# gmlwns2000/sea-attention

Measured on AMD Instinct MI355X. Metric: tokens/sec + achieved HBM GB/s, OPT-1.3B SEA T=4096 k=64, 1/2/4/8 MI355X, higher is better.
Workload: dtype bf16

## Files before the change

include/sea_hip.h:

```cpp
#ifndef SEA_HIP_H
#define SEA_HIP_H

#include <stdint.h>

#ifdef __cplusplus
extern "C" {
#endif

#define SEA_ABI_VERSION 6

enum sea_dtype { SEA_F32 = 0, SEA_F16 = 1, SEA_BF16 = 2 };

enum sea_error {
  SEA_OK = 0,
  SEA_EINVAL = -1,
  SEA_EUNSUPPORTED = -2,
  SEA_ELAUNCH = -3
};

typedef void* sea_stream_t;

int sea_version(void);
const char* sea_last_error(void);

// ... 42 lines not shown

int sea_csr_elmul(const float* in_values, float* out_values,
                  const void* other, int dtype, const int64_t* other_strides ,
                  int64_t N, int64_t H, int64_t T_dst, int64_t T_src,
                  const void* crow, const void* col, int idx_bytes, int64_t col_stride_n,
                  sea_stream_t stream);

int sea_csr_spmm(const float* values, const void* v, int dtype,
                 int64_t N, int64_t H, int64_t T_dst, int64_t T_src, int64_t D,
                 const int64_t* v_strides ,
                 const void* crow, const void* col, int idx_bytes, int64_t col_stride_n,
                 const int32_t* head_off,
                 float* out, sea_stream_t stream);

enum sea_attn_path { SEA_ATTN_AUTO = 0, SEA_ATTN_GATHER = 1, SEA_ATTN_TILE = 2, SEA_ATTN_KEYRANGE = 3 };
int sea_sparse_attention(const void* q, const void* k, const void* v, int dtype,
                         int64_t N, int64_t H, int64_t T_dst, int64_t T_src, int64_t D,
                         const int64_t* q_strides, const int64_t* k_strides, const int64_t* v_strides,
                         const int32_t* crow, const int32_t* col, int64_t col_stride_n,
                         const int32_t* head_off,
                         const float* row_scale,
                         const void* avg, const int64_t* avg_strides,
                         const float* mix,
                         void* out, int out_dtype, const int64_t* out_strides,
                         float* probs_out, int64_t probs_stride_n,
                         const uint8_t* block_path,
                         int flags,
                         const uint32_t* bits, int64_t T_m, int is_causal, int max_k, int write_cols,
                         const int32_t* t_src_dev,
                         int64_t t_src_stride,
// ... 120 lines not shown
```

sea-attention_amd/_lib.py:

```python
import ctypes
import os
from ctypes import c_int, c_int32, c_int64, c_void_p, c_char_p, POINTER

import torch

from . import _build

SEA_F32, SEA_F16, SEA_BF16 = 0, 1, 2
ABI_VERSION = 6
_DTYPES = {torch.float32: SEA_F32, torch.float16: SEA_F16, torch.bfloat16: SEA_BF16}

_lib = None

i64 = c_int64
ptr = c_void_p
_i64p = POINTER(c_int64)

_SIGNATURES = {
    "sea_version": ([], c_int),
    "sea_last_error": ([], c_char_p),
    "sea_topk_select": ([ptr, c_int, i64, i64, i64, i64, i64, i64, i64, ptr, i64, i64, c_int, c_int,
                         ptr, ptr, ptr, ptr, ptr], c_int),
    "sea_mask_to_bits": ([ptr, c_int, i64, i64, i64, i64, i64, i64, i64, i64, c_int, c_int,
                          ptr, ptr, ptr, ptr], c_int),
# ... 46 lines not shown
    "sea_decode_append_rows": ([c_int, i64, i64, i64, i64, i64, i64, i64, i64, ptr, ptr, _i64p, _i64p, ptr, ptr, i64, i64, i64,
                                ptr, i64, ptr, i64, i64, ptr, i64, ptr, i64, ptr, ptr, ptr, i64, c_int32, c_int32, c_int32, ptr],
                               c_int),
    "sea_performer_avg_supported": ([i64, i64, c_int], c_int),
    "sea_performer_plan": ([i64, i64, i64, i64, i64, c_int, _i64p, _i64p], c_int),
}

EXPORTED_SYMBOLS = tuple(_SIGNATURES)


def library_path():
    return _build.LIB_PATH


SEA_ATTN_AUTO, SEA_ATTN_GATHER, SEA_ATTN_TILE, SEA_ATTN_KEYRANGE = 0, 1, 2, 3
SEA_OK, SEA_EINVAL, SEA_EUNSUPPORTED = 0, -1, -2


def load(build_if_missing=True):
    global _lib
    if _lib is not None:
        return _lib
    override = os.environ.get("SEA_HIP_LIB")
    if override:
        if not os.path.exists(override):
            raise RuntimeError(f"SEA_HIP_LIB={override} does not exist")
        path = override
    else:
        path = _build.LIB_PATH
        if _build.is_stale():
# ... 92 lines not shown
```

sea-attention_amd/csrc/sea_attn.hip:

```cpp
#include "sea_attn.hpp"

namespace sea {

template <typename T, typename TO, int LPR, int U, bool WP>
__global__ __launch_bounds__(256) void sparse_attn_kernel(AttnParams p) {
  constexpr int VEC = Elem<T>::VEC;
  constexpr int KPI = 64 / LPR;
  int pair, tb;
  if (!map_block(p.N * p.H, p.TB, &pair, &tb)) return;
  const int n = pair / p.H, h = pair - n * p.H;
  const int t = tb * 4 + (threadIdx.x >> 6);
  if (t >= p.T_dst) return;
  if (kernel_is_idle(p)) return;
  const int lane = threadIdx.x & 63;
  const int grp = lane / LPR, sub = lane - grp * LPR;
  const bool dact = sub * VEC < p.D;

  const T* qp = reinterpret_cast<const T*>(p.q) + n * p.qs[0] + h * p.qs[1] + t * p.qs[2] + sub * VEC;
  const T* kb = reinterpret_cast<const T*>(p.k) + n * p.ks[0] + h * p.ks[1] + sub * VEC;
  const T* vb = reinterpret_cast<const T*>(p.v) + n * p.vs[0] + h * p.vs[1] + sub * VEC;

  uint4 qraw = make_uint4(0, 0, 0, 0);
  if (dact) qraw = *reinterpret_cast<const uint4*>(qp);
  const int row_beg = p.crow[(int64_t)n * (p.T_dst + 1) + t];
// ... 84 lines not shown
      const T* ap = reinterpret_cast<const T*>(p.avg) + n * p.as[0] + h * p.as[1] + t * p.as[2] + sub * VEC;
      float af[VEC];
      unpack16<T>(*reinterpret_cast<const uint4*>(ap), af);
#pragma unroll
      for (int j = 0; j < VEC; ++j) o[j] = o[j] * a + (1.0f - a) * af[j];
    }
    TO* op = reinterpret_cast<TO*>(p.out) + n * p.os[0] + h * p.os[1] + t * p.os[2] + sub * VEC;
    store_frag<TO, VEC>(op, o);
  }
}

__device__ inline int slot_length(const AttnParams& p, int n, int h, int tn) {
  if (tn >= p.T_dst) return -1;
  const int32_t* hon = p.head_off + ((int64_t)n * p.T_dst + tn) * (p.H + 1);
  return hon[h + 1] - hon[h];
}

template <int LPR, int RPB, bool DEC = false>
__device__ inline void fused_expand(const AttnParams& p, int n, int h, int tt, bool rowok, int gi, int sub, int beg, int end,
                                    int hcol, int t_src, int* s_keys, int* lbase_out, bool* fits_out, int* total_out) {
  __shared__ int s_glen[RPB];
  const int mylen = end - beg;
  if (sub == 0) s_glen[gi] = mylen;
  __syncthreads();
  int bef = 0, tot = 0;
#pragma unroll
  for (int r = sub; r < RPB; r += LPR) {
    const int v_ = s_glen[r];
    tot += v_;
    bef += r < gi ? v_ : 0;
// ... 76 lines not shown
    }
    asm volatile("" ::"v"(sink));
  }
  __syncthreads();
}

template <bool FUSE>
__device__ inline int entry_column(const AttnParams& p, const int32_t* col, int n, int ec, int beg, const int* s_keys, int lbase, bool fits) {
  if (FUSE && fits) return s_keys[lbase + ec - beg];
  if (FUSE) return __hip_atomic_load(p.col_w + n * p.col_stride_n + ec, __ATOMIC_RELAXED, __HIP_MEMORY_SCOPE_AGENT);
  return col[ec];
}

constexpr int SEA_ATTN_WARM_ROWS = 8;

template <typename T, typename TO, int LPR, int U, bool WP, int NWB = 4, bool FUSE = false, bool DEC = false>
__global__ __launch_bounds__(NWB * 64, (FUSE && !DEC && sizeof(T) == 2 && !WP) ? 8 : 1) void sparse_attn_rows_kernel(AttnParams p) {
  static_assert(!DEC || FUSE, "the decode form is a fused form");
  constexpr int VEC = Elem<T>::VEC;
  constexpr int RPW = 64 / LPR;
  constexpr int RPB = NWB * RPW;
  int pair, tb;
  if (kernel_is_idle(p) || !map_block(p.N * p.H, p.TB, &pair, &tb)) return;
  const int n = pair / p.H;
  const int h = (pair - n * p.H + n) % p.H;
  const int lane = threadIdx.x & 63;
  const int grp = lane / LPR, sub = lane - grp * LPR;
  const int gi = (int)(threadIdx.x >> 6) * RPW + grp;
  bool rowok;
  const int t = tb * RPB + rows_by_length<LPR, RPB>(slot_length(p, n, h, tb * RPB + gi), gi, sub, &rowok);
  const bool dact = sub * VEC < p.D;
  const int tt = t < p.T_dst ? t : p.T_dst - 1;
  const int sube = dact ? sub : 0;

  const char* kbase = reinterpret_cast<const char*>(reinterpret_cast<const T*>(p.k) + n * p.ks[0] + h * p.ks[1]);
  const char* vbase = reinterpret_cast<const char*>(reinterpret_cast<const T*>(p.v) + n * p.vs[0] + h * p.vs[1]);
  const uint32_t kst = (uint32_t)p.ks[2] * (uint32_t)sizeof(T), vst = (uint32_t)p.vs[2] * (uint32_t)sizeof(T);
  const uint32_t lane_off = (uint32_t)(sube * VEC) * (uint32_t)sizeof(T);

  uint4 qraw = make_uint4(0, 0, 0, 0);
  if (dact) qraw = *reinterpret_cast<const uint4*>(reinterpret_cast<const T*>(p.q) + n * p.qs[0] + h * p.qs[1] +
                                                  (int64_t)tt * p.qs[2] + sub * VEC);
  const int row_beg = p.crow[(int64_t)n * (p.T_dst + 1) + tt];
  const int32_t* ho = p.head_off + ((int64_t)n * p.T_dst + tt) * (p.H + 1);
  const int beg = row_beg + ho[h];
// ... 135 lines not shown
}
template <> __device__ inline float tail_dot<__half>(uint32_t q, uint32_t k, float d) {
  return __builtin_amdgcn_fdot2(__builtin_bit_cast(sea_h2, q), __builtin_bit_cast(sea_h2, k), d, false);
}
template <typename T> __device__ inline void unpack2(uint32_t r, float* f);
template <> __device__ inline void unpack2<__hip_bfloat16>(uint32_t r, float* f) {
  f[0] = __uint_as_float(r << 16); f[1] = __uint_as_float(r & 0xffff0000u);
}
template <> __device__ inline void unpack2<__half>(uint32_t r, float* f) {
  const float2 t = __half22float2(__builtin_bit_cast(__half2, r));
  f[0] = t.x; f[1] = t.y;
}
template <typename TO> __device__ inline void store2(TO* dst, float a, float b) { *reinterpret_cast<uint32_t*>(dst) = pack2<TO>(a, b); }
template <> __device__ inline void store2<float>(float* dst, float a, float b) { *reinterpret_cast<float2*>(dst) = make_float2(a, b); }

template <typename T, typename TO, int U, bool WP, int NWB = 4, bool FUSE = false, bool DEC = false>
__global__ __launch_bounds__(NWB * 64) void sparse_attn_rows80_kernel(AttnParams p) {
  static_assert(!DEC || FUSE, "the decode form is a fused form");
  constexpr int LPR = 8, VEC = 8, XT = 2, DM = LPR * VEC;
  constexpr int RPW = 64 / LPR, RPB = NWB * RPW;
  int pair, tb;
  if (kernel_is_idle(p) || !map_block(p.N * p.H, p.TB, &pair, &tb)) return;
  const int n = pair / p.H;
  const int h = (pair - n * p.H + n) % p.H;
  const int lane = threadIdx.x & 63;
  const int grp = lane / LPR, sub = lane - grp * LPR;
  const int gi = (int)(threadIdx.x >> 6) * RPW + grp;
  bool rowok;
  const int t = tb * RPB + rows_by_length<LPR, RPB>(slot_length(p, n, h, tb * RPB + gi), gi, sub, &rowok);
  const int tt = t < p.T_dst ? t : p.T_dst - 1;

  const char* kbase = reinterpret_cast<const char*>(reinterpret_cast<const T*>(p.k) + n * p.ks[0] + h * p.ks[1]);
  const char* vbase = reinterpret_cast<const char*>(reinterpret_cast<const T*>(p.v) + n * p.vs[0] + h * p.vs[1]);
  const uint32_t kst = (uint32_t)p.ks[2] * (uint32_t)sizeof(T), vst = (uint32_t)p.vs[2] * (uint32_t)sizeof(T);
  const uint32_t off_m = (uint32_t)(sub * VEC) * (uint32_t)sizeof(T);
  const uint32_t off_x = (uint32_t)(DM + sub * XT) * (uint32_t)sizeof(T);

  const T* qrow = reinterpret_cast<const T*>(p.q) + n * p.qs[0] + h * p.qs[1] + (int64_t)tt * p.qs[2];
  const uint4 qraw = *reinterpret_cast<const uint4*>(qrow + sub * VEC);
  const uint32_t qx = *reinterpret_cast<const uint32_t*>(qrow + DM + sub * XT);
  const int row_beg = p.crow[(int64_t)n * (p.T_dst + 1) + tt];
  const int32_t* ho = p.head_off + ((int64_t)n * p.T_dst + tt) * (p.H + 1);
  const int beg = row_beg + ho[h];
  const int end = rowok ? row_beg + ho[h + 1] : beg;
// ... 499 lines not shown
      } else if (lpr == 8) {
        constexpr int CH = 256, DL = 64;
        hipLaunchKernelGGL((sparse_attn_decode1_kernel<T, TO, 8, false, false, WP>), dim3((unsigned)NH), dim3(256), CH * 8 + CH + CH * DL * 2, s, p);
      } else {
        constexpr int CH = 128, DL = 128;
        hipLaunchKernelGGL((sparse_attn_decode1_kernel<T, TO, 16, false, false, WP>), dim3((unsigned)NH), dim3(256), CH * 8 + CH + CH * DL * 2, s, p);
      }
      return SEA_OK;
    }
  }
  if (p.table) return SEA_EUNSUPPORTED;
  if constexpr (sizeof(T) == 2) {
    if (p.D == 80 && small) {
      const int rpb = 8 * 8;
      p.TB = (p.T_dst + rpb - 1) / rpb;
      const int64_t blocks = (int64_t)8 * ((NH + 7) / 8) * p.TB;
      if (p.bits && p.t_src_dev) {
        hipLaunchKernelGGL((sparse_attn_rows80_kernel<T, TO, 4, WP, 8, true, true>), dim3((unsigned)blocks), dim3(512), p.fuse_cap * (int)sizeof(int), s, p);
      } else if (p.bits) hipLaunchKernelGGL((sparse_attn_rows80_kernel<T, TO, 4, WP, 8, true>), dim3((unsigned)blocks), dim3(512), p.fuse_cap * (int)sizeof(int), s, p);
      else hipLaunchKernelGGL((sparse_attn_rows80_kernel<T, TO, 4, WP, 8>), dim3((unsigned)blocks), dim3(512), 0, s, p);
      return SEA_OK;
    }
  }
  if (lpr <= 16 && small) {
    const int nwb = lpr == 4 ? 4 : 8;
    const int rpb = nwb * (64 / lpr);
    p.TB = (p.T_dst + rpb - 1) / rpb;
    const int64_t blocks = (int64_t)8 * ((NH + 7) / 8) * p.TB;
    dim3 grid((unsigned)blocks), block(nwb * 64);
    if (p.bits) {
      if (lpr == 4) return SEA_EUNSUPPORTED;
      const int lds = p.fuse_cap * (int)sizeof(int);
      if (p.t_src_dev) {
        if (lpr == 8) hipLaunchKernelGGL((sparse_attn_rows_kernel<T, TO, 8, 4, WP, 8, true, true>), grid, block, lds, s, p);
        else hipLaunchKernelGGL((sparse_attn_rows_kernel<T, TO, 16, 4, WP, 8, true, true>), grid, block, lds, s, p);
        return SEA_OK;
      }
      if (lpr == 8) hipLaunchKernelGGL((sparse_attn_rows_kernel<T, TO, 8, 4, WP, 8, true>), grid, block, lds, s, p);
      else hipLaunchKernelGGL((sparse_attn_rows_kernel<T, TO, 16, 4, WP, 8, true>), grid, block, lds, s, p);
      return SEA_OK;
    }
    switch (lpr) {
      case 4: hipLaunchKernelGGL((sparse_attn_rows_kernel<T, TO, 4, 4, WP, 4>), grid, block, 0, s, p); break;
      case 8: hipLaunchKernelGGL((sparse_attn_rows_kernel<T, TO, 8, 4, WP, 8>), grid, block, 0, s, p); break;
      default: hipLaunchKernelGGL((sparse_attn_rows_kernel<T, TO, 16, 4, WP, 8>), grid, block, 0, s, p); break;
    }
    return SEA_OK;
  }
  if (p.bits) return SEA_EUNSUPPORTED;
  const int64_t blocks = (int64_t)8 * ((NH + 7) / 8) * p.TB;
  dim3 grid((unsigned)blocks), block(256);
  switch (lpr) {
// ... 53 lines not shown
  SEA_REQUIRE(dtype == SEA_F32 || dtype == SEA_F16 || dtype == SEA_BF16, SEA_EINVAL, "%s: bad dtype %d", name, dtype);
  return SEA_OK;
}

extern "C" int sea_sparse_attention(const void* q, const void* k, const void* v, int dtype, int64_t N, int64_t H,
                                    int64_t T_dst, int64_t T_src, int64_t D, const int64_t* q_strides,
                                    const int64_t* k_strides, const int64_t* v_strides, const int32_t* crow,
                                    const int32_t* col, int64_t col_stride_n, const int32_t* head_off,
                                    const float* row_scale, const void* avg, const int64_t* avg_strides,
                                    const float* mix, void* out, int out_dtype, const int64_t* out_strides,
                                    float* probs_out, int64_t probs_stride_n, const uint8_t* block_path, int flags,
                                    const uint32_t* bits, int64_t T_m, int is_causal, int max_k, int write_cols,
                                    const int32_t* t_src_dev, int64_t t_src_stride, const int32_t* block_table,
                                    int64_t table_stride, int64_t page_rows, sea_stream_t stream) {
  const char* nm = "sea_sparse_attention";
  const bool keyrange = (flags & 0xff) == SEA_ATTN_KEYRANGE;
  KeyRangeParams kr = {nullptr, 0, 0, 0};
  if (keyrange) {
    SEA_REQUIRE(bits != nullptr, SEA_EUNSUPPORTED, "%s: the key-range form is a fused form (bits is NULL)", nm);
    SEA_REQUIRE(t_src_dev == nullptr && block_table == nullptr && t_src_stride == 0, SEA_EUNSUPPORTED,
                "%s: the key-range form has no decode or paged form (t_src_dev / block_table)", nm);
    SEA_REQUIRE(write_cols == 0, SEA_EUNSUPPORTED, "%s: the key-range form writes no columns (write_cols must be 0)", nm);
    SEA_REQUIRE(N > 0 && H > 0 && T_dst > 0 && T_src > 0 && D > 0, SEA_EINVAL, "%s: bad shape", nm);
    SEA_REQUIRE(dtype == SEA_F32 ? (D == 32 || D == 64) : (D == 64 || D == 128), SEA_EUNSUPPORTED,
                "%s: the key-range form takes 16-bit D in {64, 128} or fp32 D in {32, 64} (dtype %d, D=%lld)", nm, dtype, (long long)D);
    const int64_t rk = (flags >> 16) & 0x7fff;
    SEA_REQUIRE(rk > 0, SEA_EINVAL, "%s: the key-range form needs range_keys (1 .. 32767) in bits 16..30 of flags", nm);
    const int64_t nr = (T_src + rk - 1) / rk;
    SEA_REQUIRE(nr <= 64, SEA_EUNSUPPORTED, "%s: the key-range form takes at most 64 ranges (%lld keys in ranges of %lld: %lld)", nm,
                (long long)T_src, (long long)rk, (long long)nr);
// ... 58 lines not shown
  p.crow = crow; p.col = col; p.col_stride_n = col_stride_n; p.head_off = head_off;
  p.row_scale = row_scale; p.avg = avg; p.mix = mix; p.out = out;
  p.probs = probs_out; p.probs_stride_n = probs_stride_n;
  p.sel = nullptr; p.sel_want = 0; p.TB16 = (int)((T_dst + 15) / 16);
  p.sel_count = nullptr; p.sel_total = (int)(N * H * p.TB16);
  p.sel_num = D >= 128 ? 13 : 1; p.sel_den = D >= 128 ? 20 : 2;
  p.bits = bits; p.col_w = const_cast<int32_t*>(col); p.T_m = (int)T_m; p.W = (int)((H * T_m + 31) / 32);
  p.max_k = max_k; p.is_causal = is_causal;
  p.fuse_cap = 8192;
  p.write_cols = write_cols != 0;
  p.t_src_dev = t_src_dev;
  SEA_REQUIRE(t_src_stride >= 0 && t_src_stride * N < (1ll << 31), SEA_EINVAL, "%s: bad T_src stride %lld", nm,
              (long long)t_src_stride);
  p.t_src_stride = (int)t_src_stride;
  p.table = block_table; p.table_stride = (int)table_stride; p.page_shift = block_table ? __builtin_ctzll(page_rows) : 0;
  if (t_src_dev) {
    SEA_REQUIRE(bits != nullptr && T_dst <= SEA_ATTN_WARM_ROWS, SEA_EUNSUPPORTED,
                "%s: the decode form takes T_dst <= %d rows per sequence", nm, SEA_ATTN_WARM_ROWS);
    SEA_REQUIRE(probs_out == nullptr || probs_stride_n >= col_stride_n, SEA_EINVAL,
                "%s: the decode form's probs_out needs probs_stride_n >= col_stride_n (%lld < %lld)", nm,
                (long long)probs_stride_n, (long long)col_stride_n);
  }
  if (bits) {
    SEA_REQUIRE(path != SEA_ATTN_TILE && block_path == nullptr, SEA_EUNSUPPORTED, "%s: the fused interpolation runs on the gather kernels", nm);
    SEA_REQUIRE(T_m > 0 && T_m % 32 == 0 && max_k > 0, SEA_EUNSUPPORTED, "%s: fused interpolation needs T_m %% 32 == 0", nm);
    if (t_src_dev) SEA_REQUIRE(H * T_src < (1ll << 31), SEA_EUNSUPPORTED, "%s: the decode form needs int32 ids (H*T_cap < 2^31)", nm);
    else SEA_REQUIRE(H * T_src < (1ll << 24), SEA_EUNSUPPORTED, "%s: H*T_src must stay below 2^24 (fp32-exact ids)", nm);
  }
  p.TB = (int)((T_dst + 3) / 4);
  hipStream_t s = (hipStream_t)stream;
// ... 120 lines not shown
```

sea-attention_amd/csrc/sea_attn.hpp:

```cpp
#pragma once
#include "sea_common.hpp"

namespace sea {

struct AttnParams {
  const void *q, *k, *v;
  int64_t qs[3], ks[3], vs[3];
  int N, H, T_dst, T_src, D;
  const int32_t* crow;
  const int32_t* col;
  int64_t col_stride_n;
  const int32_t* head_off;
  const float* row_scale;
  const void* avg;
  int64_t as[3];
  const float* mix;
  void* out;
  int64_t os[3];
  float* probs;
  int64_t probs_stride_n;
  const uint8_t* sel;
  int sel_want, TB16;
  const int32_t* sel_count;
  int sel_total, sel_num, sel_den;
  int TB;
  const uint32_t* bits;
  int32_t* col_w;
  int T_m, W, max_k, is_causal, fuse_cap;
  int write_cols;
  const int32_t* t_src_dev;
  int t_src_stride;
  const int32_t* table;
  int table_stride, page_shift;
};

template <typename TO, int VEC> __device__ inline void store_frag(TO* dst, const float* f);
template <> __device__ inline void store_frag<float, 4>(float* dst, const float* f) {
  *reinterpret_cast<float4*>(dst) = make_float4(f[0], f[1], f[2], f[3]);
}
template <> __device__ inline void store_frag<float, 8>(float* dst, const float* f) {
  *reinterpret_cast<float4*>(dst) = make_float4(f[0], f[1], f[2], f[3]);
  *reinterpret_cast<float4*>(dst + 4) = make_float4(f[4], f[5], f[6], f[7]);
}
template <> __device__ inline void store_frag<__hip_bfloat16, 8>(__hip_bfloat16* dst, const float* f) {
  union { uint4 u; __hip_bfloat16 h[8]; } r;
#pragma unroll
  for (int i = 0; i < 8; ++i) r.h[i] = __float2bfloat16(f[i]);
  *reinterpret_cast<uint4*>(dst) = r.u;
// ... 130 lines not shown
```

sea-attention_amd/perlin_attention/attention.py:

```python
import math
import os
import warnings
from typing import NamedTuple, Optional

import torch
import torch.nn.functional as F
from torch import nn

from ..utils import get_bench
from .config import PerlinAttentionConfig, get_default_config
from .modules import CausalConv2d, KeepRes, UpsampleFP32
from .performer import FastAttention, ProjectionUpdater
from . import ops

timer = lambda name: get_bench().region(name)
mem = lambda name: get_bench().mem_region(name)
_C8_DECLINED = set()


def _safe_to(t, d):
    return t.to(d) if isinstance(t, torch.Tensor) else t


class PerlinAttentionOutput(NamedTuple):
    loss: torch.Tensor
    context_layer: torch.Tensor
    partial_attention_probs: torch.Tensor
    partial_attention_mask: torch.Tensor
    estimated_attention_probs_m: torch.Tensor
    estimated_attention_probs: torch.Tensor
    dense_attention_probs: torch.Tensor
    key_for_score: torch.Tensor
# ... 57 lines not shown
        self.num_attention_heads = config.num_attention_heads
        self.attention_head_size = int(config.hidden_size / config.num_attention_heads)
        self.all_head_size = self.num_attention_heads * self.attention_head_size
        self._warning_messages = ""

        self.benchmarking = False
        self.context_layer_dtype = None
        self.assume_not_padded = None
        self.materialize_csr = False
        self.return_attention_probs = False
        self.lazy_attention_probs = True
        self.lazy_csr_columns = True
        self.conv_z_epilogue = False
        self.sparse_kernel = "auto"
        self.key_range: Optional[int] = None
        self.performer_segments = None
        self.force_torch_estimator = False
        self.dense_head_chunk = None
        self._fused_gates = None
        self._fused_selection = None
        self._avg_ahead = None

        d, H = self.attention_head_size, self.num_attention_heads
        pc = self.pconfig

        self.performer_nb_features = int(d * math.log(d) / pc.performer_nb_factor)
        self.performer = FastAttention(dim_heads=d, nb_features=self.performer_nb_features,
                                       causal=pc.causal, generalized_attention=pc.causal)
        self.performer_proj_updater = ProjectionUpdater(self.performer, 1000)
        if pc.attention_predictor_backend != 'performer':
# ... 722 lines not shown
                                                       mix=average_scale)
                    ctx = p2.permute(0, 2, 1, 3).reshape(N, T, H * HID).to(out_dtype)
                else:
                    ctx = torch.empty((N, T, H * HID), dtype=out_dtype, device=q.device)
                    plan = None
                    if (self.sparse_kernel == "auto" and not want_probs and qs.dtype != torch.float32
                            and HID in (64, 80, 128) and not csr.col_is_pending):
                        plan = ops.attention_plan(csr, T_M, is_causal=True)
                    if (self.key_range is not None and not want_probs and csr.col_is_pending and self.lazy_csr_columns
                            and T_SRC > self.key_range
                            and ops.keyrange_supported(qs.dtype, HID, T_M, T_SRC, int(self.key_range))):
                        res = ops.sparse_attention(qs, ks, vs, csr, row_scale=row_scale, avg=average_context_layer,
                                                   mix=average_scale, out=ctx.view(N, T, H, HID).permute(0, 2, 1, 3),
                                                   path="keyrange", range_keys=int(self.key_range))
                    else:
                        res = ops.sparse_attention(qs, ks, vs, csr, row_scale=row_scale, avg=average_context_layer,
                                                   mix=average_scale, out=ctx.view(N, T, H, HID).permute(0, 2, 1, 3),
                                                   want_probs=want_probs, path="gather" if want_probs else self.sparse_kernel,
                                                   plan=plan, keep_columns_pending=self.lazy_csr_columns and not want_probs)
                    if want_probs:
                        probs_csr = csr.with_values(res[1])
        if probs_csr is not None:
            bench.register_temp_buffer('partial_attention_probs', None, lazy=lambda: ops.flat_csr_to_dense(probs_csr, T_SRC, H))
        if self.materialize_csr:
            return ctx, (probs_csr.to_sparse_csr() if probs_csr is not None else None), csr.to_sparse_csr()
        return ctx, probs_csr, csr

    def _forward_dense(self, q, v, q_for_score, k_for_score, t_attention_predictor, probs, causal_attention_mask,
                       dst_attention_mask, attention_scores_truth, FP_MIN, T_SRC, T_M, resize_dense, head_chunk=None):
        bench = get_bench()
        N, H, T, HID = q.shape
        k_, os_ = self.pconfig.k, self.pconfig.k_oversample
        loss = 0
        with timer("mask"):
# ... 96 lines not shown
```

sea-attention_amd/perlin_attention/ops/__init__.py:

```python
from .resize_dense import resize_from_m_to_t
from .flat_csr import resize_from_m_to_t_csr
from .flat_csr import flat_csr_elmul
from .flat_csr import flat_csr_masked_bmm
from .flat_csr import flat_csr_sdbmm
from .flat_csr import flat_csr_softmax
from .flat_csr import flat_csr_to_dense
from .flat_csr import (FlatCSR, fused_interp_supported, attention_few_rows, topk_to_csr, topk_mask, sparse_attention, sparse_attention_bytes, attention_plan, plan_blocks, make_plan,
                       sparse_attention_autograd, keyrange_supported, keyrange_workspace_floats,
                       keep_table_causal, keep_table_kernel_test, z_capacity, csr_from_selection)
from .predictor import (split_layernorm, predictor_tail, cumavg, performer_value, performer_supported, performer_avg_supported,
                        performer_step, performer_plan, performer_chunk_rows,
                        split_layernorm_c8, causal_conv_c8, causal_conv_c8_z, conv_z_supported, conv_c8_f32_supported, predictor_tail_z, pack_conv_weight, to_c8, from_c8,
                        predictor_mlp, predictor_mlp_supported, predictor_tail_select,
                        predictor_tail_select_supported, clear_prep_cache, prep_generation, pinned_prep, LazyTensor, realize,
                        decode_stage, c8_window_shift, decode_fork, decode_fork_staging_bytes, decode_cnn_tail_select, decode_cnn_supported, decode_cnn_emits, decode_tail_select_supported, DECODE_PREDICTOR_LENGTHS,
                        decode_gather_rows, decode_append_rows)
```

sea-attention_amd/perlin_attention/ops/flat_csr.py:

```python
import math
from ctypes import c_void_p, c_int64
from typing import Optional

import torch

from ... import _lib


def _p(t: Optional[torch.Tensor]):
    return c_void_p(t.data_ptr()) if t is not None else c_void_p(0)


class FlatCSR:

    def __init__(self, crow, col, head_off, H, T_src, bits=None, row_nnz=None, vals=None):
        self.crow, self._col, self.head_off = crow, col, head_off
        self.H, self.T_src = H, T_src
        self.bits, self.row_nnz = bits, row_nnz
        self.vals = vals
        self.N, self.T_dst = crow.shape[0], crow.shape[1] - 1
        self._wire = None
        self._pending = None
        self.t_src_dev = None

# ... 210 lines not shown
    return lanes in (8, 16) and D % vec == 0 and T_m % 32 == 0


def keyrange_supported(dtype, D: int, T_m: int, T_src: Optional[int] = None, range_keys: Optional[int] = None) -> bool:
    if not (D in ((32, 64) if dtype == torch.float32 else (64, 128)) and T_m % 32 == 0):
        return False
    if range_keys is None:
        return True
    return 1 <= range_keys <= 32767 and (T_src is None or -(-T_src // range_keys) <= KEYRANGE_MAX_RANGES)


def keyrange_workspace_floats(N: int, H: int, T_dst: int, D: int, n_ranges: int) -> int:
    return N * H * n_ranges * T_dst * (D + 2)


_BWD_WS = {}
_KEYRANGE_WS = {}


def _keyrange_workspace(N: int, stride: int, device) -> torch.Tensor:
    return _stream_workspace(_KEYRANGE_WS, N * stride * 4, device).view(torch.float32).view(N, stride)


def _bwd_workspace(nbytes: int, device) -> torch.Tensor:
    return _stream_workspace(_BWD_WS, nbytes, device)


def _stream_workspace(cache: dict, nbytes: int, device) -> torch.Tensor:
    if torch.cuda.is_current_stream_capturing():
        return torch.empty((nbytes,), dtype=torch.uint8, device=device)
    key = (device.type, device.index, torch.cuda.current_stream(device).cuda_stream)
    ws = cache.get(key)
    if ws is None or ws.numel() < nbytes:
        cache[key] = ws = torch.empty((nbytes,), dtype=torch.uint8, device=device)
    return ws[:nbytes]


def clear_bwd_workspace():
    _BWD_WS.clear()
    _KEYRANGE_WS.clear()


class _SparseAttentionFn(torch.autograd.Function):
    backward_form = "gather"

    @staticmethod
    def forward(ctx, q, k, v, csr):
        with torch.no_grad():
            out, probs = sparse_attention(q.detach(), k.detach(), v.detach(), csr, want_probs=True, path="gather")
        ctx.save_for_backward(q, k, v, probs, out)
        ctx.csr = csr
        return out

    @staticmethod
    def backward(ctx, dout):
# ... 49 lines not shown
    _lib.require_gpu(csr.bits)
    nb = csr.N * csr.H * ((csr.T_dst + 15) // 16)
    buf = torch.empty((((nb + 3) & ~3) + 4,), dtype=torch.uint8, device=csr.bits.device)
    _lib.check(lib.sea_attention_plan(_p(csr.bits), csr.N, csr.H, csr.T_dst, csr.T_src, int(T_m), int(is_causal),
                                      float(entries_per_tile), _p(buf), _lib.stream_ptr()), "sea_attention_plan")
    return buf


@_lib.device_guarded
def sparse_attention(q, k, v, csr: FlatCSR, row_scale: Optional[torch.Tensor] = None,
                     avg: Optional[torch.Tensor] = None, mix: Optional[torch.Tensor] = None,
                     out: Optional[torch.Tensor] = None, out_dtype: Optional[torch.dtype] = None,
                     path: str = "auto", want_probs: bool = False, row_tiles: int = 0, key_window: int = 0,
                     plan: Optional[torch.Tensor] = None, fuse_emit: bool = True, keep_columns_pending: bool = False,
                     block_table: Optional[torch.Tensor] = None, range_keys: Optional[int] = None,
                     probs_out: Optional[torch.Tensor] = None):
    lib = _lib.load()
    want_probs = want_probs or probs_out is not None
    if probs_out is not None:
        _lib.require_gpu(probs_out)
        assert (probs_out.dtype == torch.float32 and probs_out.dim() == 2 and probs_out.shape[0] == csr.N
                and probs_out.shape[1] >= csr._col.shape[1] and probs_out.stride(1) == 1
                and (csr.N == 1 or probs_out.stride(0) >= csr._col.stride(0))), "probs_out: fp32 (N, >= z_cap), feature stride 1"
    _lib.require_gpu(q, k, v, csr.crow, block_table)
    keyrange = path == "keyrange"
    if keyrange:
        why = None
        if range_keys is None or not 1 <= int(range_keys) <= 32767:
            why = f"range_keys must be 1 .. 32767 (got {range_keys})"
        elif not csr.col_is_pending:
            why = "it takes a handle whose columns are pending (topk_to_csr / csr_from_selection with defer_emit=True)"
        elif want_probs or plan is not None:
# ... 34 lines not shown
        assert k.shape == (N, H, T_src, D) and v.shape == (N, H, T_src, D)
    assert q.dtype == k.dtype == v.dtype
    assert (csr.N, csr.T_dst, csr.H, csr.T_src) == (N, T_dst, H, T_src)
    if out is None:
        out = torch.empty((N, H, T_dst, D), dtype=out_dtype or torch.float32, device=q.device)
    assert out.shape == (N, H, T_dst, D) and out.stride(-1) == 1
    if row_scale is not None:
        assert row_scale.dtype == torch.float32 and row_scale.shape == (N, H, T_dst) and row_scale.is_contiguous()
    if mix is not None:
        assert avg is not None and avg.shape == (N, H, T_dst, D) and avg.dtype == q.dtype
        assert mix.dtype == torch.float32 and mix.shape == (N, H, T_dst) and mix.is_contiguous()
    if plan is not None:
        nb_ = N * H * ((T_dst + 15) // 16)
        assert plan.dtype == torch.uint8 and plan.numel() == ((nb_ + 3) & ~3) + 4 and plan.is_contiguous()

    def launch(col, probs, block_path, flags, bits=None, T_m=0, is_causal=0, max_k=0, write_cols=1, t_src_dev=None):
        return lib.sea_sparse_attention(
            _p(q), _p(k), _p(v), _lib.dtype_code(q.dtype), N, H, T_dst, T_src, D,
            _lib.strides3(q), _lib.strides3(k), _lib.strides3(v),
            _p(csr.crow), _p(col), col.stride(0), _p(csr.head_off),
            _p(row_scale), _p(avg), _lib.strides3(avg) if avg is not None else None, _p(mix),
            _p(out), _lib.dtype_code(out.dtype), _lib.strides3(out),
            _p(probs), probs.stride(0) if probs is not None else 0, _p(block_path), flags,
            _p(bits), T_m, is_causal, max_k, write_cols, _p(t_src_dev), csr.t_src_stride if t_src_dev is not None else 0,
            _p(block_table), table_stride, page_rows, _lib.stream_ptr())

    if keyrange:
        T_m_, max_k_, causal_, _emit = csr._pending
        n_ranges = -(-T_src // int(range_keys))
        stride = (keyrange_workspace_floats(1, H, T_dst, D, n_ranges) + 3) & ~3
        ws = _keyrange_workspace(N, stride, q.device)
        _lib.check(launch(csr._col, ws, None, _lib.SEA_ATTN_KEYRANGE | (int(range_keys) << 16), csr.bits, T_m_, int(causal_),
                          max_k_, 0), "sea_sparse_attention")
        return out
    if fused:
        T_m_, max_k_, causal_, _emit = csr._pending
        raw_col = csr._col
        probs = probs_out
        if want_probs and probs is None:
            probs = torch.zeros(raw_col.shape, dtype=torch.float32, device=q.device)
        rc = launch(raw_col, probs, None, _lib.SEA_ATTN_GATHER, csr.bits, T_m_, int(causal_), max_k_,
                    0 if keep_columns_pending else 1, csr.t_src_dev)
        if rc == 0:
            if not keep_columns_pending:
                csr._pending = None
            return (out, probs) if want_probs else out
        if rc != _lib.SEA_EUNSUPPORTED or paged:
            _lib.check(rc, "sea_sparse_attention")
    probs = probs_out
    if want_probs and probs is None:
        probs = torch.zeros(csr.col.shape, dtype=torch.float32, device=q.device)
    flags = _PATHS[path] | ((int(row_tiles) & 0xf) << 8)
    if key_window:
        assert key_window & (key_window - 1) == 0, "key_window is a power of two"
        flags |= (int(key_window).bit_length() - 1) << 12
    block_path = plan if (plan is not None and path == "auto" and not want_probs) else None
    _lib.check(launch(csr.col, probs, block_path, flags), "sea_sparse_attention")
# ... 172 lines not shown
```

Measured before the change: 15.56 million.

## Sort attention rows by CSR length within pools before fused gather kernels

Adds a pre-pass kernel that counting-sorts query rows by their sparse row length within pools of up to 1024 rows per head, writing a uint16 order table. The fused gather attention kernels then take rows from these pools in sorted order rather than from fixed 64-row tiles, so rows of similar length share a workgroup and wave imbalance drops. This replaces the earlier per-workgroup local reordering. It costs an extra kernel launch and a workspace allocation, and it is on by default (pool 512) for bf16/fp16 with head sizes 64 and 128.

```diff
diff --git a/include/sea_hip.h b/include/sea_hip.h
--- a/include/sea_hip.h
+++ b/include/sea_hip.h
@@ -80,6 +80,7 @@
                  float* out, sea_stream_t stream);
 
 enum sea_attn_path { SEA_ATTN_AUTO = 0, SEA_ATTN_GATHER = 1, SEA_ATTN_TILE = 2, SEA_ATTN_KEYRANGE = 3 };
+enum { SEA_ATTN_ROW_POOL_SHIFT = 4 };
 int sea_sparse_attention(const void* q, const void* k, const void* v, int dtype,
                          int64_t N, int64_t H, int64_t T_dst, int64_t T_src, int64_t D,
                          const int64_t* q_strides, const int64_t* k_strides, const int64_t* v_strides,
diff --git a/sea-attention_amd/_lib.py b/sea-attention_amd/_lib.py
--- a/sea-attention_amd/_lib.py
+++ b/sea-attention_amd/_lib.py
@@ -84,6 +84,7 @@
 
 
 SEA_ATTN_AUTO, SEA_ATTN_GATHER, SEA_ATTN_TILE, SEA_ATTN_KEYRANGE = 0, 1, 2, 3
+SEA_ATTN_ROW_POOL_SHIFT = 4
 SEA_OK, SEA_EINVAL, SEA_EUNSUPPORTED = 0, -1, -2
 
 
diff --git a/sea-attention_amd/csrc/sea_attn.hip b/sea-attention_amd/csrc/sea_attn.hip
--- a/sea-attention_amd/csrc/sea_attn.hip
+++ b/sea-attention_amd/csrc/sea_attn.hip
@@ -122,6 +122,61 @@
   if (tn >= p.T_dst) return -1;
   const int32_t* hon = p.head_off + ((int64_t)n * p.T_dst + tn) * (p.H + 1);
   return hon[h + 1] - hon[h];
+}
+
+constexpr int SEA_ATTN_ORDER_BINS = 512;
+__global__ __launch_bounds__(1024) void attn_row_order_kernel(AttnParams p) {
+  constexpr int BINS = SEA_ATTN_ORDER_BINS;
+  __shared__ int s_bin[BINS];
+  __shared__ int s_top[1024];
+  const int tid = threadIdx.x, pool = p.pool_rows;
+  const int pl = (int)blockIdx.x % p.pools, pair = (int)blockIdx.x / p.pools;
+  const int n = pair / p.H, h = pair - n * p.H;
+  for (int b = tid; b < BINS; b += blockDim.x) s_bin[b] = 0;
+  const bool mine = tid < pool;
+  const int len = mine ? slot_length(p, n, h, pl * pool + tid) : -1;
+  const int bin = len + 1 < BINS - 1 ? len + 1 : BINS - 1;
+  if (mine) s_top[tid] = bin == BINS - 1 ? len : -1;
+  __syncthreads();
+  if (mine) atomicAdd(&s_bin[bin], 1);
+  __syncthreads();
+  if (tid < 64) {
+    constexpr int PER = BINS / 64;
+    int c[PER], sum = 0;
+#pragma unroll
+    for (int i = 0; i < PER; ++i) { c[i] = s_bin[BINS - 1 - (tid * PER + i)]; sum += c[i]; }
+    int start = wave_incl_scan(sum) - sum;
+#pragma unroll
+    for (int i = 0; i < PER; ++i) { s_bin[BINS - 1 - (tid * PER + i)] = start; start += c[i]; }
+  }
+  __syncthreads();
+  if (!mine) return;
+  int slot;
+  if (bin == BINS - 1) {
+    slot = 0;
+    for (int r = 0; r < pool; ++r) {
+      const int o = s_top[r];
+      slot += (o > len || (o == len && r < tid)) ? 1 : 0;
+    }
+  } else {
+    slot = atomicAdd(&s_bin[bin], 1);
+  }
+  uint16_t* ord = const_cast<uint16_t*>(p.order) + n * p.order_stride_n + ((int64_t)h * p.pools + pl) * pool;
+  ord[slot] = (uint16_t)tid;
+}
+
+template <int LPR, int RPB>
+__device__ inline bool pooled_row(const AttnParams& p, int n, int h, int tb, int grp, int* t, bool* rowok) {
+  constexpr int RPW = 64 / LPR;
+  const int nb = p.pool_rows / RPB;
+  const int pl = tb / nb, b = tb - pl * nb;
+  const int rows = min(p.pool_rows, p.T_dst - pl * p.pool_rows);
+  if (b * RPW >= rows) return false;
+  const int slot = (((int)threadIdx.x >> 6) * nb + b) * RPW + grp;
+  const uint16_t* ord = p.order + n * p.order_stride_n + ((int64_t)h * p.pools + pl) * p.pool_rows;
+  *t = pl * p.pool_rows + (int)ord[slot];
+  *rowok = *t < p.T_dst;
+  return true;
 }
 
 template <int LPR, int RPB, bool DEC = false>
@@ -228,9 +283,10 @@
 
 constexpr int SEA_ATTN_WARM_ROWS = 8;
 
-template <typename T, typename TO, int LPR, int U, bool WP, int NWB = 4, bool FUSE = false, bool DEC = false>
+template <typename T, typename TO, int LPR, int U, bool WP, int NWB = 4, bool FUSE = false, bool DEC = false, bool ORD = false>
 __global__ __launch_bounds__(NWB * 64, (FUSE && !DEC && sizeof(T) == 2 && !WP) ? 8 : 1) void sparse_attn_rows_kernel(AttnParams p) {
   static_assert(!DEC || FUSE, "the decode form is a fused form");
+  static_assert(!ORD || (FUSE && !DEC && !WP), "rows are dealt from pools in the fused inference form only");
   constexpr int VEC = Elem<T>::VEC;
   constexpr int RPW = 64 / LPR;
   constexpr int RPB = NWB * RPW;
@@ -242,7 +298,12 @@
   const int grp = lane / LPR, sub = lane - grp * LPR;
   const int gi = (int)(threadIdx.x >> 6) * RPW + grp;
   bool rowok;
-  const int t = tb * RPB + rows_by_length<LPR, RPB>(slot_length(p, n, h, tb * RPB + gi), gi, sub, &rowok);
+  int t;
+  if constexpr (ORD) {
+    if (!pooled_row<LPR, RPB>(p, n, h, tb, grp, &t, &rowok)) return;
+  } else {
+    t = tb * RPB + rows_by_length<LPR, RPB>(slot_length(p, n, h, tb * RPB + gi), gi, sub, &rowok);
+  }
   const bool dact = sub * VEC < p.D;
   const int tt = t < p.T_dst ? t : p.T_dst - 1;
   const int sube = dact ? sub : 0;
@@ -408,9 +469,10 @@
 template <typename TO> __device__ inline void store2(TO* dst, float a, float b) { *reinterpret_cast<uint32_t*>(dst) = pack2<TO>(a, b); }
 template <> __device__ inline void store2<float>(float* dst, float a, float b) { *reinterpret_cast<float2*>(dst) = make_float2(a, b); }
 
-template <typename T, typename TO, int U, bool WP, int NWB = 4, bool FUSE = false, bool DEC = false>
+template <typename T, typename TO, int U, bool WP, int NWB = 4, bool FUSE = false, bool DEC = false, bool ORD = false>
 __global__ __launch_bounds__(NWB * 64) void sparse_attn_rows80_kernel(AttnParams p) {
   static_assert(!DEC || FUSE, "the decode form is a fused form");
+  static_assert(!ORD || (FUSE && !DEC && !WP), "rows are dealt from pools in the fused inference form only");
   constexpr int LPR = 8, VEC = 8, XT = 2, DM = LPR * VEC;
   constexpr int RPW = 64 / LPR, RPB = NWB * RPW;
   int pair, tb;
@@ -421,7 +483,12 @@
   const int grp = lane / LPR, sub = lane - grp * LPR;
   const int gi = (int)(threadIdx.x >> 6) * RPW + grp;
   bool rowok;
-  const int t = tb * RPB + rows_by_length<LPR, RPB>(slot_length(p, n, h, tb * RPB + gi), gi, sub, &rowok);
+  int t;
+  if constexpr (ORD) {
+    if (!pooled_row<LPR, RPB>(p, n, h, tb, grp, &t, &rowok)) return;
+  } else {
+    t = tb * RPB + rows_by_length<LPR, RPB>(slot_length(p, n, h, tb * RPB + gi), gi, sub, &rowok);
+  }
   const int tt = t < p.T_dst ? t : p.T_dst - 1;
 
   const char* kbase = reinterpret_cast<const char*>(reinterpret_cast<const T*>(p.k) + n * p.ks[0] + h * p.ks[1]);
@@ -951,6 +1018,16 @@
     if (p.D == 80 && small) {
       const int rpb = 8 * 8;
       p.TB = (p.T_dst + rpb - 1) / rpb;
+      if constexpr (!WP) {
+        if (p.order) {
+          if (p.pool_rows % rpb) return SEA_EINVAL;
+          p.TB = p.pools * (p.pool_rows / rpb);
+          const int64_t pblocks = (int64_t)8 * ((NH + 7) / 8) * p.TB;
+          hipLaunchKernelGGL(attn_row_order_kernel, dim3((unsigned)(NH * p.pools)), dim3(p.pool_rows < 64 ? 64 : p.pool_rows), 0, s, p);
+          hipLaunchKernelGGL((sparse_attn_rows80_kernel<T, TO, 4, false, 8, true, false, true>), dim3((unsigned)pblocks), dim3(512), p.fuse_cap * (int)sizeof(int), s, p);
+          return SEA_OK;
+        }
+      }
       const int64_t blocks = (int64_t)8 * ((NH + 7) / 8) * p.TB;
       if (p.bits && p.t_src_dev) {
         hipLaunchKernelGGL((sparse_attn_rows80_kernel<T, TO, 4, WP, 8, true, true>), dim3((unsigned)blocks), dim3(512), p.fuse_cap * (int)sizeof(int), s, p);
@@ -973,6 +1050,17 @@
         else hipLaunchKernelGGL((sparse_attn_rows_kernel<T, TO, 16, 4, WP, 8, true, true>), grid, block, lds, s, p);
         return SEA_OK;
       }
+      if constexpr (!WP) {
+        if (p.order) {
+          if (p.pool_rows % rpb) return SEA_EINVAL;
+          p.TB = p.pools * (p.pool_rows / rpb);
+          const dim3 pgrid((unsigned)((int64_t)8 * ((NH + 7) / 8) * p.TB));
+          hipLaunchKernelGGL(attn_row_order_kernel, dim3((unsigned)(NH * p.pools)), dim3(p.pool_rows < 64 ? 64 : p.pool_rows), 0, s, p);
+          if (lpr == 8) hipLaunchKernelGGL((sparse_attn_rows_kernel<T, TO, 8, 4, false, 8, true, false, true>), pgrid, block, lds, s, p);
+          else hipLaunchKernelGGL((sparse_attn_rows_kernel<T, TO, 16, 4, false, 8, true, false, true>), pgrid, block, lds, s, p);
+          return SEA_OK;
+        }
+      }
       if (lpr == 8) hipLaunchKernelGGL((sparse_attn_rows_kernel<T, TO, 8, 4, WP, 8, true>), grid, block, lds, s, p);
       else hipLaunchKernelGGL((sparse_attn_rows_kernel<T, TO, 16, 4, WP, 8, true>), grid, block, lds, s, p);
       return SEA_OK;
@@ -1056,6 +1144,41 @@
                                     const int32_t* t_src_dev, int64_t t_src_stride, const int32_t* block_table,
                                     int64_t table_stride, int64_t page_rows, sea_stream_t stream) {
   const char* nm = "sea_sparse_attention";
+  int pool_log2 = (flags >> SEA_ATTN_ROW_POOL_SHIFT) & 0xf;
+  flags &= ~(0xf << SEA_ATTN_ROW_POOL_SHIFT);
+  const uint16_t* order = nullptr;
+  int64_t order_stride_n = 0;
+  if (pool_log2) {
+    const char* rp = "the row-pool form";
+    SEA_REQUIRE((flags & 0xff) != SEA_ATTN_KEYRANGE && (flags & 0xff) != SEA_ATTN_TILE, SEA_EUNSUPPORTED,
+                "%s: %s deals the rows of the fused gather kernels: the key-range and tile paths have none (path %d)", nm, rp, flags & 0xff);
+    SEA_REQUIRE(bits != nullptr, SEA_EUNSUPPORTED, "%s: %s is a fused form (bits is NULL)", nm, rp);
+    SEA_REQUIRE(t_src_dev == nullptr && block_table == nullptr && t_src_stride == 0, SEA_EUNSUPPORTED,
+                "%s: %s has no decode or paged form (t_src_dev / block_table)", nm, rp);
+    SEA_REQUIRE(probs_out == nullptr, SEA_EUNSUPPORTED, "%s: %s writes no per-entry probabilities (probs_out must be NULL)", nm, rp);
+    SEA_REQUIRE(N > 0 && H > 0 && T_dst > 0 && T_src > 0 && D > 0, SEA_EINVAL, "%s: bad shape", nm);
+    if (N * H * T_dst <= SEA_ATTN_FEW_ROWS) {
+      pool_log2 = 0;
+      block_path = nullptr;
+      probs_stride_n = 0;
+    }
+  }
+  if (pool_log2) {
+    const char* rp = "the row-pool form";
+    const int64_t pool = 1ll << pool_log2;
+    SEA_REQUIRE(pool <= 1024, SEA_EUNSUPPORTED, "%s: %s takes pools of at most 1024 rows (got %lld)", nm, rp, (long long)pool);
+    const int64_t rpb = (dtype == SEA_F32 ? D > 32 : (D > 64 && D != 80)) ? 32 : 64;
+    SEA_REQUIRE(pool % rpb == 0, SEA_EUNSUPPORTED, "%s: %s needs a pool that is a multiple of the %lld rows of a workgroup (got %lld)",
+                nm, rp, (long long)rpb, (long long)pool);
+    const int64_t pools = (T_dst + pool - 1) / pool, need = H * pools * pool;
+    SEA_REQUIRE(block_path != nullptr && aligned16(block_path) && probs_stride_n >= need, SEA_EINVAL,
+                "%s: %s needs a 16-byte aligned uint16 workspace in block_path with probs_stride_n >= %lld elements per batch "
+                "item (got %lld)", nm, rp, (long long)need, (long long)probs_stride_n);
+    order = reinterpret_cast<const uint16_t*>(block_path);
+    order_stride_n = probs_stride_n;
+    block_path = nullptr;
+    probs_stride_n = 0;
+  }
   const bool keyrange = (flags & 0xff) == SEA_ATTN_KEYRANGE;
   KeyRangeParams kr = {nullptr, 0, 0, 0};
   if (keyrange) {
@@ -1144,6 +1267,8 @@
               (long long)t_src_stride);
   p.t_src_stride = (int)t_src_stride;
   p.table = block_table; p.table_stride = (int)table_stride; p.page_shift = block_table ? __builtin_ctzll(page_rows) : 0;
+  p.order = order; p.order_stride_n = order_stride_n;
+  p.pool_rows = order ? 1 << pool_log2 : 0; p.pools = order ? (int)((T_dst + p.pool_rows - 1) / p.pool_rows) : 0;
   if (t_src_dev) {
     SEA_REQUIRE(bits != nullptr && T_dst <= SEA_ATTN_WARM_ROWS, SEA_EUNSUPPORTED,
                 "%s: the decode form takes T_dst <= %d rows per sequence", nm, SEA_ATTN_WARM_ROWS);
diff --git a/sea-attention_amd/csrc/sea_attn.hpp b/sea-attention_amd/csrc/sea_attn.hpp
--- a/sea-attention_amd/csrc/sea_attn.hpp
+++ b/sea-attention_amd/csrc/sea_attn.hpp
@@ -32,6 +32,9 @@
   int t_src_stride;
   const int32_t* table;
   int table_stride, page_shift;
+  const uint16_t* order;
+  int64_t order_stride_n;
+  int pool_rows, pools;
 };
 
 template <typename TO, int VEC> __device__ inline void store_frag(TO* dst, const float* f);
diff --git a/sea-attention_amd/perlin_attention/attention.py b/sea-attention_amd/perlin_attention/attention.py
--- a/sea-attention_amd/perlin_attention/attention.py
+++ b/sea-attention_amd/perlin_attention/attention.py
@@ -16,6 +16,8 @@
 timer = lambda name: get_bench().region(name)
 mem = lambda name: get_bench().mem_region(name)
 _C8_DECLINED = set()
+ATTENTION_ROW_POOL: Optional[int] = 512
+ATTENTION_ROW_POOL_HEAD_SIZES = (64, 128)
 
 
 def _safe_to(t, d):
@@ -103,6 +105,7 @@
         self.conv_z_epilogue = False
         self.sparse_kernel = "auto"
         self.key_range: Optional[int] = None
+        self.attention_row_pool: Optional[int] = ATTENTION_ROW_POOL
         self.performer_segments = None
         self.force_torch_estimator = False
         self.dense_head_chunk = None
@@ -855,10 +858,15 @@
                                                    mix=average_scale, out=ctx.view(N, T, H, HID).permute(0, 2, 1, 3),
                                                    path="keyrange", range_keys=int(self.key_range))
                     else:
+                        row_pool = self.attention_row_pool
+                        if row_pool is not None and not (qs.dtype != torch.float32 and HID in ATTENTION_ROW_POOL_HEAD_SIZES
+                                                         and ops.row_pool_supported(qs.dtype, HID, int(row_pool))):
+                            row_pool = None
                         res = ops.sparse_attention(qs, ks, vs, csr, row_scale=row_scale, avg=average_context_layer,
                                                    mix=average_scale, out=ctx.view(N, T, H, HID).permute(0, 2, 1, 3),
                                                    want_probs=want_probs, path="gather" if want_probs else self.sparse_kernel,
-                                                   plan=plan, keep_columns_pending=self.lazy_csr_columns and not want_probs)
+                                                   plan=plan, keep_columns_pending=self.lazy_csr_columns and not want_probs,
+                                                   row_pool=row_pool)
                     if want_probs:
                         probs_csr = csr.with_values(res[1])
         if probs_csr is not None:
diff --git a/sea-attention_amd/perlin_attention/ops/__init__.py b/sea-attention_amd/perlin_attention/ops/__init__.py
--- a/sea-attention_amd/perlin_attention/ops/__init__.py
+++ b/sea-attention_amd/perlin_attention/ops/__init__.py
@@ -7,6 +7,7 @@
 from .flat_csr import flat_csr_to_dense
 from .flat_csr import (FlatCSR, fused_interp_supported, attention_few_rows, topk_to_csr, topk_mask, sparse_attention, sparse_attention_bytes, attention_plan, plan_blocks, make_plan,
                        sparse_attention_autograd, keyrange_supported, keyrange_workspace_floats,
+                       row_pool_supported, row_pool_workspace, row_pool_workspace_elems,
                        keep_table_causal, keep_table_kernel_test, z_capacity, csr_from_selection)
 from .predictor import (split_layernorm, predictor_tail, cumavg, performer_value, performer_supported, performer_avg_supported,
                         performer_step, performer_plan, performer_chunk_rows,
diff --git a/sea-attention_amd/perlin_attention/ops/flat_csr.py b/sea-attention_amd/perlin_attention/ops/flat_csr.py
--- a/sea-attention_amd/perlin_attention/ops/flat_csr.py
+++ b/sea-attention_amd/perlin_attention/ops/flat_csr.py
@@ -248,8 +248,27 @@
     return N * H * n_ranges * T_dst * (D + 2)
 
 
+ROW_POOL_MAX = 1024
+
+
+def row_pool_supported(dtype, D: int, row_pool: int) -> bool:
+    vec = 4 if dtype == torch.float32 else 8
+    rpb = 64 if (D == 80 and vec == 8) or D <= 8 * vec else 32
+    return row_pool >= rpb and row_pool <= ROW_POOL_MAX and row_pool & (row_pool - 1) == 0
+
+
+def row_pool_workspace_elems(N: int, H: int, T_dst: int, row_pool: int) -> int:
+    return N * H * -(-T_dst // row_pool) * row_pool
+
+
 _BWD_WS = {}
 _KEYRANGE_WS = {}
+_ROW_POOL_WS = {}
+
+
+def row_pool_workspace(N: int, H: int, T_dst: int, row_pool: int, device) -> torch.Tensor:
+    per = row_pool_workspace_elems(1, H, T_dst, row_pool)
+    return _stream_workspace(_ROW_POOL_WS, N * per * 2, device).view(torch.int16).view(N, H, per // H)
 
 
 def _keyrange_workspace(N: int, stride: int, device) -> torch.Tensor:
@@ -273,6 +292,7 @@
 def clear_bwd_workspace():
     _BWD_WS.clear()
     _KEYRANGE_WS.clear()
+    _ROW_POOL_WS.clear()
 
 
 class _SparseAttentionFn(torch.autograd.Function):
@@ -352,8 +372,11 @@
                      path: str = "auto", want_probs: bool = False, row_tiles: int = 0, key_window: int = 0,
                      plan: Optional[torch.Tensor] = None, fuse_emit: bool = True, keep_columns_pending: bool = False,
                      block_table: Optional[torch.Tensor] = None, range_keys: Optional[int] = None,
-                     probs_out: Optional[torch.Tensor] = None):
-    lib = _lib.load()
+                     row_pool: Optional[int] = None, probs_out: Optional[torch.Tensor] = None):
+    lib = _lib.load()
+    if row_pool is not None and not row_pool_supported(q.dtype, q.shape[-1], int(row_pool)):
+        raise ValueError(f"sparse_attention(row_pool={row_pool}): a power of two up to {ROW_POOL_MAX} and a multiple of the rows a "
+                         f"workgroup walks (64 for rows of 8 lanes, 32 for rows of 16; got {q.dtype}, d = {q.shape[-1]})")
     want_probs = want_probs or probs_out is not None
     if probs_out is not None:
         _lib.require_gpu(probs_out)
@@ -418,14 +441,18 @@
         nb_ = N * H * ((T_dst + 15) // 16)
         assert plan.dtype == torch.uint8 and plan.numel() == ((nb_ + 3) & ~3) + 4 and plan.is_contiguous()
 
-    def launch(col, probs, block_path, flags, bits=None, T_m=0, is_causal=0, max_k=0, write_cols=1, t_src_dev=None):
+    def launch(col, probs, block_path, flags, bits=None, T_m=0, is_causal=0, max_k=0, write_cols=1, t_src_dev=None, order=None):
+        if order is not None:
+            block_path, ws_stride = order, order.stride(0)
+        else:
+            ws_stride = probs.stride(0) if probs is not None else 0
         return lib.sea_sparse_attention(
             _p(q), _p(k), _p(v), _lib.dtype_code(q.dtype), N, H, T_dst, T_src, D,
             _lib.strides3(q), _lib.strides3(k), _lib.strides3(v),
             _p(csr.crow), _p(col), col.stride(0), _p(csr.head_off),
             _p(row_scale), _p(avg), _lib.strides3(avg) if avg is not None else None, _p(mix),
             _p(out), _lib.dtype_code(out.dtype), _lib.strides3(out),
-            _p(probs), probs.stride(0) if probs is not None else 0, _p(block_path), flags,
+            _p(probs), ws_stride, _p(block_path), flags,
             _p(bits), T_m, is_causal, max_k, write_cols, _p(t_src_dev), csr.t_src_stride if t_src_dev is not None else 0,
             _p(block_table), table_stride, page_rows, _lib.stream_ptr())
 
@@ -443,8 +470,12 @@
         probs = probs_out
         if want_probs and probs is None:
             probs = torch.zeros(raw_col.shape, dtype=torch.float32, device=q.device)
-        rc = launch(raw_col, probs, None, _lib.SEA_ATTN_GATHER, csr.bits, T_m_, int(causal_), max_k_,
-                    0 if keep_columns_pending else 1, csr.t_src_dev)
+        flags, order = _lib.SEA_ATTN_GATHER, None
+        if row_pool is not None and not (decode_form or paged or want_probs):
+            flags |= (int(row_pool).bit_length() - 1) << _lib.SEA_ATTN_ROW_POOL_SHIFT
+            order = row_pool_workspace(N, H, T_dst, int(row_pool), q.device)
+        rc = launch(raw_col, probs, None, flags, csr.bits, T_m_, int(causal_), max_k_,
+                    0 if keep_columns_pending else 1, csr.t_src_dev, order)
         if rc == 0:
             if not keep_columns_pending:
                 csr._pending = None
```

New measurement: 15.92 million, median of 6. +2.3%, better.
